# gregorgebhardt/gym-kilobots

Measured on AMD Instinct MI355X. Metric: kilobot-steps/sec, higher is better.
Workload: dtype f32

## Files before the change

### gym_kilobots_amd/csrc/kb_regsolve_bins.inc

```
{
    constexpr int KRB = KB_KREG_BINS;
    const bool solving = (int)__builtin_amdgcn_readfirstlane(wave) < nsolve;
    unsigned ra[KRB], rb[KRB], rm[KRB];
    float racc[KRB], rnx[KRB], rny[KRB];
    const unsigned WOFF = 8u * (unsigned)(NB - 5);
    char *const velB = reinterpret_cast<char *>(vel), *const posB = reinterpret_cast<char *>(pos);
#define RB_WALL(j) (ra[j] >= WOFF)
#define RB_WALLIDX(j) ((int)((ra[j] - WOFF) >> 3))
#define RB_VEL(off) (*reinterpret_cast<float2 *>(velB + (off)))
#define RB_POS(off) (*reinterpret_cast<float2 *>(posB + (off)))
#define RB_C(j) ((int)(rm[j] & 0xFFFu))
#define RB_DEPTH(j) ((int)((rm[j] >> 12) & 0x1FFu))
#define RB_FLIP(j) (((rm[j] >> 21) & 1u) != 0u)
#define RB_ISL(j) ((int)(rm[j] >> 22))
#pragma unroll
    for (int j = 0; j < KRB; ++j) { ra[j] = 0u; rb[j] = 0u; rm[j] = 0u; racc[j] = 0.0f; rnx[j] = 1.0f; rny[j] = 0.0f; }
    unsigned long long slotLevels[KRB];
    int dlo[KRB], dhi[KRB];
#pragma unroll
    for (int j = 0; j < KRB; ++j) { slotLevels[j] = 0ull; dlo[j] = 1; dhi[j] = 0; }
    int maxD = 0;
    unsigned mycnt = 0;
    const float nm_bb = p.nm_bb, nm_wb = p.nm_wb;
    const int DUMMY = NB - 1;
#ifdef KB_SOLVER_PRIO
    __builtin_amdgcn_s_setprio(KB_SOLVER_PRIO);
#endif
    if (solving) {
        unsigned mybase = 0;
        for (int w = 0; w < wave; ++w) mybase += misc[M_WCNT + w];
        mycnt = misc[M_WCNT + wave];
        unsigned lk[KRB];
        unsigned lp[KRB];
        int rdepth[KRB];
#define RB_A(j) ((int)(lp[j] & 0xFFFFu))
#define RB_B(j) ((int)(lp[j] >> 16))
        unsigned mlo = 0, mhi = 0;
#pragma unroll
        for (int j = 0; j < KRB; ++j) {
            const unsigned idx = lane + 64u * j;
            lk[j] = 0u; lp[j] = 0u; rdepth[j] = 0;
            if (idx < mycnt) {
                const unsigned c = lOrder[mybase + idx];
                const unsigned pr = lPair[c], inf = lInfo[c];
                const unsigned cls = inf & 0x7Fu, r = (inf >> 8) & 0xFFu;
                lp[j] = pr;
                unsigned key = cls * RK + (r < RK - 1 ? r : RK - 1);
                if (SLEEP && !active[parent[pr >> 16]]) key = 63u;
                else {
                    if (key < 32u) mlo |= 1u << key; else mhi |= 1u << (key - 32u);
                    if (r >= RK - 1) atomicMax(&bkMaxRank[wave * NUM_CLS + cls], r);
                }
                lk[j] = key | (r << 8) | (c << 16) | 0x80000000u;
            }
        }
        mlo = wave_or(mlo); mhi = wave_or(mhi);
        const unsigned long long keymask = ((unsigned long long)mhi << 32) | mlo;
        wave_sync();
#ifdef KB_PROFILE
        if (tid == 0) { atomicAdd(&KB_PROF(8), (unsigned)__popcll(keymask)); atomicAdd(&KB_PROF(11), 1u); }
#endif
        KB_STAMP_PRE(19);
        unsigned *bodyDepth = islCnt;
        {
            auto depth_round = [&](unsigned key_, int r_) __attribute__((always_inline)) {
                int ia[KRB], ib[KRB];
                unsigned da[KRB], db[KRB];
                bool on[KRB];
#pragma unroll
                for (int j = 0; j < KRB; ++j) {
                    on[j] = (lk[j] >> 31) && (lk[j] & 63u) == key_ && (r_ < 0 || (int)((lk[j] >> 8) & 0xFFu) == r_);
                    ia[j] = (on[j] && RB_A(j) < WALL_CODE) ? RB_A(j) : DUMMY;
                    ib[j] = on[j] ? RB_B(j) : DUMMY;
                    da[j] = bodyDepth[ia[j]]; db[j] = bodyDepth[ib[j]];
                }
#pragma unroll
                for (int j = 0; j < KRB; ++j) {
                    const unsigned d = max((on[j] && RB_A(j) < WALL_CODE) ? da[j] : 0u, db[j]) + 1u;
                    if (on[j]) {
                        rdepth[j] = (int)d;
                        bodyDepth[ib[j]] = d;
                        if (RB_A(j) < WALL_CODE) bodyDepth[ia[j]] = d;
                    }
                }
                wave_sync();
            };
            for (unsigned long long m_ = keymask; m_; m_ &= m_ - 1) {
                const unsigned key_ = (unsigned)__builtin_ctzll(m_);
                if ((key_ % RK) < RK - 1) depth_round(key_, -1);
                else {
                    const int maxr_ = (int)bkMaxRank[wave * NUM_CLS + key_ / RK];
                    for (int r_ = RK - 1; r_ <= maxr_; ++r_) depth_round(key_, r_);
                }
            }
        }
#pragma unroll
        for (int j = 0; j < KRB; ++j) maxD = max(maxD, rdepth[j]);
        maxD = (int)wave_umax((unsigned)maxD);
        KB_STAMP_PRE(20);
        if (mycnt > 64u) {
            unsigned base_ = 0;
            for (int d_ = SLEEP ? 0 : 1; d_ <= maxD; ++d_) {
#pragma unroll
                for (int j = 0; j < KRB; ++j) {
                    const bool is = (lk[j] >> 31) && rdepth[j] == d_;
                    const unsigned long long m_ = __ballot(is);
                    if (is) {
                        const unsigned at = mybase + base_ + (unsigned)__popcll(m_ & ((1ull << lane) - 1ull));
                        lOrder[at] = (unsigned short)((lk[j] >> 16) & 0xFFFu);
                        lCbk[at] = (unsigned short)d_;
                    }
                    base_ += (unsigned)__popcll(m_);
                }
            }
            wave_sync();
#pragma unroll
            for (int j = 0; j < KRB; ++j)
                if (lk[j] >> 31) { lk[j] = (lk[j] & 0x8000FFFFu) | ((unsigned)lOrder[mybase + lane + 64u * j] << 16); rdepth[j] = lCbk[mybase + lane + 64u * j]; }
        }
        KB_STAMP_PRE(21);
#pragma unroll
        for (int j = 0; j < KRB; ++j) {
            const unsigned long long mine = (lk[j] >> 31) ? 1ull << min(rdepth[j], 63) : 0ull;
            const unsigned lo = wave_or((unsigned)mine), hi = wave_or((unsigned)(mine >> 32));
            slotLevels[j] = ((unsigned long long)hi << 32) | (unsigned long long)lo;
            const unsigned long long lv = slotLevels[j] >> 1;
            dlo[j] = lv ? (int)__builtin_ctzll(lv) + 1 : 1;
            dhi[j] = lv ? ((lv >> 62) ? maxD : 64 - (int)__builtin_clzll(lv)) : 0;
        }
#pragma unroll
        for (int j = 0; j < KRB; ++j) {
            ra[j] = 0u; rb[j] = 0u; rm[j] = 0u;
            if (lk[j] >> 31) {
                const unsigned c = (lk[j] >> 16) & 0xFFFu;
                const unsigned pr = lPair[c], inf = lInfo[c];
                const int a = (int)(pr & 0xFFFFu), b = (int)(pr >> 16);
                const bool flip = (inf & 0x80u) != 0u;
                ra[j] = a >= WALL_CODE ? WOFF + 8u * (unsigned)(a - WALL_CODE) : 8u * (unsigned)a;
                rb[j] = 8u * (unsigned)b;
                racc[j] = lAcc[c];
                rm[j] = c | ((unsigned)rdepth[j] << 12) | (flip ? 1u << 21 : 0u) | (parent[b] << 22);
                if (a >= WALL_CODE) {
                    float dist, nx, ny;
                    wall_geom(p, a - WALL_CODE, pos[b].x, pos[b].y, dist, nx, ny);
                    if (flip) { nx = -nx; ny = -ny; }
                    rnx[j] = nx; rny[j] = ny;
                } else {
                    const float dx = pos[b].x - pos[a].x, dy = pos[b].y - pos[a].y;
                    const float dd = dx * dx + dy * dy;
                    if (dd > B2_EPSILON * B2_EPSILON) {
                        const float len = sqrtf(dd);
                        const float inv = 1.0f / len;
                        rnx[j] = dx * inv; rny[j] = dy * inv;
                    }
                }
            }
        }
#undef RB_A
#undef RB_B
#ifdef KB_PROFILE
        if (lane == 0) atomicMax(&misc[M_PROF], (unsigned)maxD);
        if (tid == 0) atomicAdd(&KB_PROF(M_PROF_DEPTH), (unsigned)maxD);
        KB_STAMP(7);
#endif
    }
    KB_ABLATE_EXIT(9);
#define RB_ON(j) (RB_DEPTH(j) == d_)
    if (solving) {
#pragma unroll
        for (int j = 0; j < KRB; ++j) {
            for (int d_ = dlo[j]; d_ <= dhi[j]; ++d_) {
                if (RB_ON(j)) {
                    const float2 va = RB_VEL(ra[j]), vb = RB_VEL(rb[j]);
                    const float Px = racc[j] * rnx[j], Py = racc[j] * rny[j];
                    const float ima = RB_WALL(j) ? 0.0f : p.im_bot;
                    RB_VEL(ra[j]) = make_float2(va.x - ima * Px, va.y - ima * Py);
                    RB_VEL(rb[j]) = make_float2(vb.x + p.im_bot * Px, vb.y + p.im_bot * Py);
                }
                wave_sync();
            }
        }
        KB_STAMP_PRE(29);
    }
    KB_ABLATE_EXIT(10);
    if (solving) {
        for (int it = 0; it < p.vel_iters; ++it) {
#pragma unroll
            for (int j = 0; j < KRB; ++j) {
                for (int d_ = dlo[j]; d_ <= dhi[j]; ++d_) {
                    if (RB_ON(j)) {
                        const float2 va = RB_VEL(ra[j]), vb = RB_VEL(rb[j]);
                        const bool wallA = RB_WALL(j);
                        const float nx = rnx[j], ny = rny[j];
                        const float ima = wallA ? 0.0f : p.im_bot, imb = p.im_bot;
                        const float dvx = vb.x - va.x, dvy = vb.y - va.y;
                        const float vn = dvx * nx + dvy * ny;
                        float lambda = -((wallA ? nm_wb : nm_bb) * vn);
                        const float accOld = racc[j];
                        const float newimp = fmaxf(accOld + lambda, 0.0f);
                        lambda = newimp - accOld;
                        racc[j] = newimp;
                        const float Px = lambda * nx, Py = lambda * ny;
                        RB_VEL(ra[j]) = make_float2(va.x - ima * Px, va.y - ima * Py);
                        RB_VEL(rb[j]) = make_float2(vb.x + imb * Px, vb.y + imb * Py);
                    }
                    wave_sync();
                }
            }
        }
        KB_STAMP_PRE(30);
    }
#ifdef KB_SOLVER_PRIO
    __builtin_amdgcn_s_setprio(0);
#endif
    __syncthreads();
    KB_STAMP(4);
    KB_RETID();
    KB_ABLATE_EXIT(11);
#ifdef KB_PROFILE
    if (tid == 0) atomicAdd(&KB_PROF(9), misc[M_PROF]);
#endif
    if (solving) {
#pragma unroll
        for (int j = 0; j < KRB; ++j)
            if (lane + 64u * j < mycnt) lAcc[RB_C(j)] = racc[j];
    }
#pragma unroll
    for (int q = 0; q < BPT; ++q) {
        const int b_ = tid + q * nt;
        if (b_ >= N) continue;
        const int b = ms[q];
        float vxx = vel[b].x, vyy = vel[b].y, ww = bw[q];
        startX[b] = pos[b].x; startY[b] = pos[b].y;
        const float tx = h * vxx, ty = h * vyy;
        if (tx * tx + ty * ty > B2_MAX_TRANSLATION_SQ) {
            const float ratio = B2_MAX_TRANSLATION / sqrtf(tx * tx + ty * ty);
            vxx *= ratio; vyy *= ratio;
        }
        const float rot = h * ww;
        if (rot * rot > B2_MAX_ROTATION_SQ) {
            const float ratio = B2_MAX_ROTATION / fabsf(rot);
            ww *= ratio;
        }
        pos[b].x += h * vxx; pos[b].y += h * vyy;
        th[q] += h * ww;
        vel[b].x = vxx; vel[b].y = vyy; bw[q] = ww;
        if (SLEEP) islWave[b] = (unsigned char)((active[b] ? 2 : 0) | (p.pos_iters <= 0 ? 1 : 0));
    }
    __syncthreads();
    KB_STAMP(5);
    KB_RETID();
    KB_ABLATE_EXIT(12);
    if (solving) {
#ifdef KB_SOLVER_PRIO
        __builtin_amdgcn_s_setprio(KB_SOLVER_PRIO);
#endif
        for (int it = 0; it < p.pos_iters; ++it) {
            unsigned char *act = active + (it & 1) * NB, *nxt = active + ((it + 1) & 1) * NB;
            bool viol = false;
            bool ron[KRB];
#pragma unroll
            for (int j = 0; j < KRB; ++j) ron[j] = (lane + 64u * j < mycnt) && act[RB_ISL(j)] != 0;
#pragma unroll
            for (int j = 0; j < KRB; ++j) {
                for (int d_ = dlo[j]; d_ <= dhi[j]; ++d_) {
                    if (ron[j] && RB_ON(j)) {
                    const bool wallA = RB_WALL(j);
                    const int isl = RB_ISL(j);
                    float nx, ny, sep;
                    const float ima = wallA ? 0.0f : p.im_bot, imb = p.im_bot;
                    const float2 pb = RB_POS(rb[j]);
                    const float bx = pb.x, by = pb.y;
                    float axx = 0.0f, ayy = 0.0f;
                    if (wallA) {
                        float dist, wx, wy;
                        wall_geom(p, RB_WALLIDX(j), bx, by, dist, wx, wy);
                        nx = RB_FLIP(j) ? -wx : wx; ny = RB_FLIP(j) ? -wy : wy;
                        const float along = RB_FLIP(j) ? -dist : dist;
                        sep = along - B2_POLYGON_RADIUS - p.r_bot;
                    } else {
                        const float2 pa = RB_POS(ra[j]);
                        axx = pa.x; ayy = pa.y;
                        const float dx = bx - axx, dy = by - ayy;
                        const float dd = dx * dx + dy * dy;
                        if (__builtin_expect(__builtin_amdgcn_ballot_w64(!kb_exact_guard(dd)) == 0ull, 1)) {
                            const float len = kb_sqrt_refine(dd, __builtin_amdgcn_sqrtf(dd), __builtin_amdgcn_rsqf(dd));
                            const float inv = kb_rcp_refine(len, __builtin_amdgcn_rcpf(len));
                            nx = dx * inv; ny = dy * inv;
                        } else {
                            const float len = sqrtf(dd);
                            nx = dx; ny = dy;
                            if (!(len < B2_EPSILON)) { const float inv = 1.0f / len; nx = dx * inv; ny = dy * inv; }
                        }
                        sep = (dx * nx + dy * ny) - p.r_bot - p.r_bot;
                    }
                    if (sep < -3.0f * B2_LINEAR_SLOP) { nxt[isl] = 1; viol = true; if (SLEEP && it == p.pos_iters - 1) islWave[isl] = 3; }
                    const float C = kb_clampf(B2_BAUMGARTE * (sep + B2_LINEAR_SLOP), -B2_MAX_LINEAR_CORRECTION, 0.0f);
                    const float K = ima + imb;
                    const float imp = __builtin_expect(p.exact_div, 1) ? kb_div_const(-C, K, wallA ? p.y_wb : p.y_bb) : (K > 0.0f ? -C / K : 0.0f);
                    const float Px = imp * nx, Py = imp * ny;
                    if (!wallA) RB_POS(ra[j]) = make_float2(axx - ima * Px, ayy - ima * Py);
                    RB_POS(rb[j]) = make_float2(bx + imb * Px, by + imb * Py);
                    }
                    wave_sync();
                }
            }
#ifdef KB_PROFILE
            if (tid == 0) atomicAdd(&KB_PROF(10), 1u);
#endif
            if (!__any(viol)) break;
#pragma unroll
            for (int j = 0; j < KRB; ++j) if (lane + 64u * j < mycnt) act[RB_ISL(j)] = 0;
            wave_sync();
        }
        KB_STAMP_PRE(24);
#ifdef KB_SOLVER_PRIO
        __builtin_amdgcn_s_setprio(0);
#endif
    }
#undef RB_WALL
#undef RB_WALLIDX
#undef RB_VEL
#undef RB_POS
#undef RB_C
#undef RB_DEPTH
#undef RB_FLIP
#undef RB_ISL
#undef RB_ON
}
```

### gym_kilobots_amd/csrc/kb_step_kernel.h

```cpp
#pragma once
#include <utility>

#include "kb_common.h"
#include "kb_objects.h"

namespace kb {

template <int DRIVE_MODE, int LIGHT_TYPE, bool OBJ, int FN = 0, int TIER = 0, bool POLY = true, bool SENSE = true, bool SLEEP = false>
__global__ void __launch_bounds__(TIER == 1 ? 64 : 64 * KB_MAX_WAVES, (TIER == 1 || TIER == 3) ? 2 : ((TIER == 2 || (FN != 0 && !OBJ)) ? KB_COMPACT_WAVES_PER_SIMD : KB_MIN_WAVES_PER_SIMD)) kb_step_kernel(const Params p) {
    constexpr bool WIDE = TIER == 1 || TIER == 3;
    constexpr bool BINS = !OBJ;
    constexpr int KRX = BINS ? KB_KREG_BINS : KREG;
    constexpr bool PAR_DS = FN != 0 && BINS;
    static_assert(!SLEEP || FN == 0 || !OBJ, "the fixed-size instantiations with objects do not carry the sleep state");
    extern __shared__ __align__(16) unsigned char smem[];
    int e = blockIdx.x;
    int tid = threadIdx.x;
    const int nt = FN ? 64 * KB_MAX_WAVES : (int)blockDim.x;
    int lane = tid & 63, wave = tid >> 6;
    const int wave_s = __builtin_amdgcn_readfirstlane(wave);
    const int nw = nt >> 6;
    const int nsolve = BINS ? (nw >= KB_NSOLVE_DIV ? nw / KB_NSOLVE_DIV : 1) : nw;
    const int N = FN ? FN : p.N, NP = FN ? ((FN + 3) & ~3) : p.NP, S = p.S;
    size_t o = (size_t)e * N;
// ... 947 lines not shown
                        int rbase = 0;
                        for (unsigned a2 = head[hix(cell)]; a2 != (unsigned)EMPTY16; a2 = nextb[a2])
                            if ((int)a2 < a && (!hashed || (int)cellOf[a2] == cell)) rbase += (int)((dirCnt[a2] >> (6 * k)) & 63u);
                        int j = 0;
                        if (((dc >> (6 * k)) & 63u) > 1u) {
                            const int oc = (cy + dir_dy(k)) * p.gw + (cx + dir_dx(k));
                            for (unsigned b2 = head[hix(oc)]; b2 != (unsigned)EMPTY16; b2 = nextb[b2]) {
                                if (b2 >= b || (k == 0 && (int)b2 <= a) || (hashed && (int)cellOf[b2] != oc)) continue;
                                const float2 pb2 = pos[b2];
                                const float ex = pb2.x - ax, ey = pb2.y - ay;
                                if (!(ex * ex + ey * ey > rr2)) j++;
                            }
                        }
                        r = rbase + j;
                        slot = sbase + j;
                        acc = ws_find(a, b);
                        if (acc < 0.0f) acc = ws_find((int)b, (unsigned)a);
                        unsigned ra = a, rb = b;
                        for (;;) {
                            while (true) { unsigned t = lds_load_relaxed<PAR_DS>(&parent[ra]); if (t == ra) break; ra = t; }
                            while (true) { unsigned t = lds_load_relaxed<PAR_DS>(&parent[rb]); if (t == rb) break; rb = t; }
                            if (ra == rb) break;
                            if (ra < rb) { unsigned t = ra; ra = rb; rb = t; }
                            if (atomicCAS(&parent[ra], ra, rb) == ra) break;
                        }
                    }
                    if (acc < 0.0f) acc = 0.0f;
                    if (slot >= S) slot = 255;
                    if (r > 255) { r = 255; atomicOr(&misc[M_STATUS], 4u); }
                    sInfo[c] = (unsigned)cls | ((unsigned)r << 8) | ((unsigned)slot << 16) | fixbits;
                    sAcc[c] = acc;
                }
            };
            if (big) label_pass(gPair, gInfo, gAcc); else label_pass(lPair, lInfo, lAcc);
            KB_STAMP_PRE(18);
            __syncthreads();
            KB_STAMP(2);
            KB_RETID();

        }

        if (SLEEP) {
#pragma unroll
            for (int q = 0; q < BPT; ++q) {
                const int b = tid + q * nt;
                if (b >= N) continue;
                const int cnt = wsCnt[b], off = wsOff[b];
                for (int s_ = 0; s_ < cnt && off + s_ < p.cap; ++s_) {
                    const float a_ = oldInLds ? oldAcc[off + s_] : g.ws_acc[wo + off + s_];
                    if (a_ < 0.0f) continue;
                    unsigned key = oldInLds ? (unsigned)oldKey[off + s_] : g.ws_key[wo + off + s_];
                    if (!oldInLds) key = key >= KEY_OBJ ? OBJ_CODE + (key - KEY_OBJ) : (key >= KEY_WALL ? WALL_CODE + (key - KEY_WALL) : key);
                    if (key >= (unsigned)WALL_CODE) continue;
                    if (slp[q] < 0.0f) slp[q] = 0.0f;
                    if (key >= (unsigned)OBJ_CODE) {
                        if (OBJ) { const int m_ = ot_body(objTab + (key - OBJ_CODE) * OT_WORDS); if (objSlp[m_] < 0.0f) objSlp[m_] = 0.0f; }
                    } else atomicOr(&misc[M_WAKE + (key >> 5)], 1u << (key & 31u));
                }
            }
            __syncthreads();
#pragma unroll
            for (int q = 0; q < BPT; ++q) {
                const int b = tid + q * nt;
                if (b < N && slp[q] < 0.0f && ((misc[M_WAKE + (b >> 5)] >> (b & 31)) & 1u)) slp[q] = 0.0f;
            }
        }
        for (int b = tid; b < N; b += nt) {
            unsigned r = b;
            while (true) { unsigned t = lds_load_relaxed<PAR_DS>(&parent[r]); if (t == r) break; r = t; }
            parent[b] = r;
            islCnt[b] = 0;
            islWave[b] = (unsigned char)((unsigned)b % (unsigned)nsolve);
            if (!BINS) head[hix(cellOf[b])] = EMPTY16;
            if (!SLEEP) active[b] = 1;
            active[NB + b] = 0;
            if (!BINS && SENSE && p.sense_s > 0 && drive) g.nbr_count[o + b] = (unsigned)newOff[b];
        }
        if (tid < 64) bkStart[tid] = 0;
        if (tid < 32) bkFill[tid] = 0;
        if (tid < M) {
            const int b = N + tid;
            unsigned r = b;
            while (true) { unsigned t = lds_load_relaxed<PAR_DS>(&parent[r]); if (t == r) break; r = t; }
            parent[b] = r;
            islCnt[b] = 0;
            islWave[b] = (unsigned char)((unsigned)b % (unsigned)nw);
            if (!SLEEP) active[b] = 1;
            active[NB + b] = 0;
        }
        if (SLEEP && !BINS) {
#pragma unroll
            for (int q = 0; q < BPT; ++q) {
                const int b = tid + q * nt;
                if (b < N && !(slp[q] < 0.0f)) active[parent[b]] = 1;
            }
            if (tid < M && !(objSlp[tid] < 0.0f)) active[parent[N + tid]] = 1;
        }
        if (BINS) __syncthreads();
        else newTotal = block_scan_u8(wsCntNew, newOff, NP, wsum, tid);
        if (SLEEP && BINS) {
#pragma unroll
            for (int q = 0; q < BPT; ++q) {
                const int b = tid + q * nt;
                if (b < N && !(slp[q] < 0.0f)) active[parent[ms[q]]] = 1;
            }
        }
        const bool newInLds = BINS ? !big : newTotal <= (unsigned)capL_;
        if (OBJ && wave == 0) {
            unsigned root = 0;
            const bool on = lane < NMC && mcTouch;
            if (on) { root = parent[mci(ox, MC_B, lane)]; mci_set(ox, MC_ISL, lane, (int)root); }
        }
        KB_STAMP(14);
        KB_RETID();
        KB_ABLATE_EXIT(7);
        const bool wcntDead = BINS && nw > 1 && p.solver_mode == 0;
        auto census = [&](const unsigned *sPair) __attribute__((always_inline)) {
            for (int c = tid; c < ncon; c += nt) {
                const unsigned root = parent[sPair[c] >> 16];
                const unsigned n = atomicAdd(&islCnt[root], 1u) + 1u;
                if (n > (unsigned)GIANT_ISLAND) atomicMax(&misc[M_MAXISL], n);
                if (!wcntDead) atomicAdd(&misc[M_WCNT + islWave[root]], 1u);
            }
        };
        if (big) census(gPair); else census(lPair);
        __syncthreads();
        unsigned maxw = 0;
        for (int w = 0; w < nw; ++w) maxw = max(maxw, misc[M_WCNT + w]);
        bool coopForced = misc[M_MAXISL] > (unsigned)GIANT_ISLAND || p.solver_mode == 2 || p.solver_mode == 4;
        bool coop = coopForced || nw == 1;
        if (!coop && !big && p.solver_mode == 0) {
            unsigned *szSum = bkStart, *szPre = bkStart + 32, *szFill = bkFill;
            for (int b = tid; b < N + M; b += nt) {
                if (parent[b] != (unsigned)b) continue;
                const unsigned cnt_ = islCnt[b];
                if (cnt_ != 0) atomicAdd(&szSum[32u - min(cnt_, 32u)], cnt_);
            }
            __syncthreads();
            if (wave == 0) {
                const unsigned v_ = lane < 32 ? szSum[lane] : 0u;
                const unsigned incl = wave_incl_scan(v_);
                if (lane < 32) szPre[lane] = incl - v_;
                if (lane < nw) misc[M_WCNT + lane] = 0;
            }
            __syncthreads();
            unsigned chunk = 60u;
            if ((unsigned)ncon > 60u * (unsigned)(nw - 1) + 124u) chunk = ((unsigned)ncon - 124u + (unsigned)nw - 2u) / (unsigned)(nw - 1);
            if (BINS) chunk = ((unsigned)ncon + (unsigned)nsolve - 1u) / (unsigned)nsolve;
            for (int b = tid; b < N + M; b += nt) {
                if (parent[b] != (unsigned)b) continue;
                const unsigned cnt_ = islCnt[b];
                if (cnt_ == 0) continue;
                const unsigned q_ = 32u - min(cnt_, 32u);
                const unsigned at = szPre[q_] + atomicAdd(&szFill[q_], cnt_);
                const unsigned w_ = min(at / max(chunk, 1u), (unsigned)nsolve - 1u);
                islWave[b] = (unsigned char)w_;
                atomicAdd(&misc[M_WCNT + w_], cnt_);
            }
            __syncthreads();
            maxw = 0;
            for (int w = 0; w < nw; ++w) maxw = max(maxw, misc[M_WCNT + w]);
        }
        bool reg = !coopForced && !big && maxw <= 64u * KRX && p.solver_mode == 0;
        if (!coop && !big && maxw > 64u * KRX && p.solver_mode == 0) {
            unsigned short *bigList = bkList;
            __syncthreads();
            if (tid < nw) misc[M_WCNT + tid] = 0;
            if (tid == 0) misc[M_TOTAL] = 0;
            __syncthreads();
            for (int b = tid; b < N + M; b += nt) {
                if (parent[b] != (unsigned)b) continue;
                const unsigned cnt_ = islCnt[b];
                if (cnt_ == 0) continue;
                unsigned slot_ = 64u;
                if (cnt_ >= (unsigned)BIG_ISLAND) slot_ = atomicAdd(&misc[M_TOTAL], 1u);
                if (slot_ < 64u) bigList[slot_] = (unsigned short)b;
                else atomicAdd(&misc[M_WCNT + islWave[b]], cnt_);
            }
            __syncthreads();
            if (wave == 0) {
                const int nb = (int)min(misc[M_TOTAL], 64u);
                const unsigned root = lane < nb ? (unsigned)bigList[lane] : 0u;
                const unsigned size = lane < nb ? islCnt[root] : 0u;
                int rank = 0;
                for (int j = 0; j < nb; ++j) {
                    const unsigned sj = __shfl(size, j), rj = __shfl(root, j);
                    if (sj > size || (sj == size && rj < root)) rank++;
                }
                unsigned load = lane < nsolve ? misc[M_WCNT + lane] : 0u;
                int myWave = 0;
                for (int r = 0; r < nb; ++r) {
                    const int src = __builtin_ctzll(__ballot(lane < nb && rank == r));
                    const unsigned sz = __shfl(size, src);
                    unsigned key = lane < nsolve ? ((load << 4) | (unsigned)lane) : 0xFFFFFFFFu;
                    for (int d = 8; d >= 1; d >>= 1) key = min(key, __shfl_xor(key, d));
                    const int wmin = (int)(__shfl(key, 0) & 15u);
                    if (lane == wmin) load += sz;
                    if (lane == src) myWave = wmin;
                }
                if (lane < nb) islWave[root] = (unsigned char)myWave;
                if (lane < nsolve) misc[M_WCNT + lane] = load;
            }
            __syncthreads();
            maxw = 0;
            for (int w = 0; w < nw; ++w) maxw = max(maxw, misc[M_WCNT + w]);
            reg = maxw <= 64u * KRX;
        }
        if (BINS && nw > 1 && !reg && p.solver_mode == 0) { coopForced = true; coop = true; }
        if (OBJ && wave == 0) {
            const bool on = lane < NMC && mcTouch && (!SLEEP || active[mci(ox, MC_ISL, lane)] != 0);
            const unsigned w_ = on ? (unsigned)islWave[mci(ox, MC_ISL, lane)] : 0u;
            for (int w = 0; w < nw; ++w) {
                const unsigned long long mk = __ballot(on && (int)w_ == w);
                if (lane == 0) mcMask[w] = mk;
            }
            const unsigned long long all = __ballot(on);
            if (lane == 0) mcMask[nw] = all;
        }
        auto mc_warm_pass = [&](unsigned long long mask, bool leader) __attribute__((always_inline)) {
            if (leader) for (unsigned long long m_ = mask; m_; m_ &= m_ - 1) mc_warm_start(ox, __builtin_ctzll(m_));
        };
        auto mc_velocity_pass = [&](unsigned long long mask, bool leader) __attribute__((always_inline)) {
            if (leader) for (unsigned long long m_ = mask; m_; m_ &= m_ - 1) mc_solve_velocity(ox, __builtin_ctzll(m_));
        };
        auto mc_position_pass = [&](unsigned long long mask, bool leader, const unsigned char *act, unsigned char *nxt, bool lastIt) __attribute__((always_inline)) -> bool {
            bool viol = false;
            if (leader)
                for (unsigned long long m_ = mask; m_; m_ &= m_ - 1) {
                    const int t = __builtin_ctzll(m_);
                    const int isl = mci(ox, MC_ISL, t);
                    if (!act[isl]) continue;
                    const float minSep = mc_solve_position(ox, t, B2_BAUMGARTE);
                    if (minSep < -3.0f * B2_LINEAR_SLOP) { nxt[isl] = 1; viol = true; if (SLEEP && lastIt) islWave[isl] = 3; }
                }
            return viol;
        };
        auto mc_clear_flags = [&](unsigned long long mask, bool leader, unsigned char *act) __attribute__((always_inline)) {
            if (leader) for (unsigned long long m_ = mask; m_; m_ &= m_ - 1) act[mci(ox, MC_ISL, __builtin_ctzll(m_))] = 0;
        };
        auto mc_store = [&]() __attribute__((always_inline)) {
            if (OBJ && wave == 0 && lane < NMC) {
                int owner, col;
                mc_candidate(F, lane, owner, col);
                float *dst = owsMine + (owner * KB_OWS_COLS + col) * KB_OWS_WORDS;
                float o[KB_OWS_WORDS] = {-1.0f, -1.0f, -1.0f, -1.0f, -1.0f, -1.0f};
                if (mcTouch) {
                    const int cnt = (mci(ox, MC_TYPE, lane) >> 2) & 3, ids = mci(ox, MC_ID, lane);
                    o[0] = (float)(ids & 255); o[1] = mcf(ox, MC_NI0, lane); o[2] = mcf(ox, MC_TI0, lane);
                    if (cnt == 2) { o[3] = (float)((ids >> 8) & 255); o[4] = mcf(ox, MC_NI1, lane); o[5] = mcf(ox, MC_TI1, lane); }
                }
#pragma unroll
                for (int k = 0; k < KB_OWS_WORDS; ++k) dst[k] = o[k];
            }
        };
        auto bucket_sort = [&](const unsigned *sPair, const unsigned *sInfo, unsigned short *cbk,
                               unsigned short *order) __attribute__((always_inline)) {
            const int W = coop ? 1 : nw;
            for (int b = tid; b < N + M; b += nt) islCnt[b] = 0;
            for (int k = tid; k < W * BK_PER_WAVE; k += nt) { bkStart[k] = 0; bkFill[k] = 0; }
            for (int k = tid; k < W * NUM_CLS; k += nt) bkMaxRank[k] = 0;
            if (tid == 0) bkStart[W * BK_PER_WAVE] = 0;
            __syncthreads();
            for (int c = tid; c < ncon; c += nt) {
                const unsigned root = parent[sPair[c] >> 16];
                if (SLEEP && !active[root]) { cbk[c] = EMPTY16; continue; }
                const int w = coop ? 0 : (int)islWave[root];
                const unsigned inf = sInfo[c];
                const int cls = inf & 0x7F, r = (inf >> 8) & 0xFF;
                const int bk = (w * NUM_CLS + cls) * RK + (r < RK - 1 ? r : RK - 1);
                cbk[c] = (unsigned short)bk;
                atomicAdd(&bkStart[bk], 1u);
                if (r >= RK - 1) atomicMax(&bkMaxRank[w * NUM_CLS + cls], (unsigned)r);
            }
            __syncthreads();
            if (wave == 0) {
                const int nb = W * BK_PER_WAVE;
                const int chunk = (nb + 63) / 64;
                const int s0 = lane * chunk, e0 = min(nb, s0 + chunk);
                unsigned sum = 0;
                for (int i = s0; i < e0; ++i) sum += bkStart[i];
                const unsigned incl = wave_incl_scan(sum);
                unsigned run = incl - sum;
                for (int i = s0; i < e0; ++i) { unsigned v = bkStart[i]; bkStart[i] = run; run += v; }
                if (lane == 63) bkStart[nb] = incl;
            }
            __syncthreads();
            for (int c = tid; c < ncon; c += nt) {
                const int bk = cbk[c];
                if (SLEEP && bk == (int)EMPTY16) continue;
                order[bkStart[bk] + atomicAdd(&bkFill[bk], 1u)] = (unsigned short)c;
            }
            if (wave < W) {
                const int base = wave * BK_PER_WAVE;
                const bool ne = lane < BK_PER_WAVE && bkStart[base + lane + 1] > bkStart[base + lane];
                const unsigned long long m = __ballot(ne);
                if (ne) bkList[base + __popcll(m & ((1ull << lane) - 1ull))] = (unsigned short)(base + lane);
                if (lane == 0) nList[wave] = (unsigned char)__popcll(m);
            }
            __syncthreads();
        };
        if (reg) {
            for (int b = tid; b < N + M; b += nt) islCnt[b] = 0;
            if (tid < nw * NUM_CLS) bkMaxRank[tid] = 0;
            for (int c = tid; c < ncon; c += nt) {
                const unsigned w = islWave[parent[lPair[c] >> 16]];
                unsigned base = 0;
                for (unsigned w2 = 0; w2 < w; ++w2) base += misc[M_WCNT + w2];
                lOrder[base + atomicAdd(&misc[M_WFILL + w], 1u)] = (unsigned short)c;
            }
            __syncthreads();
        } else if (big) bucket_sort(gPair, gInfo, gCbk, gOrder);
        else bucket_sort(lPair, lInfo, lCbk, lOrder);
        KB_STAMP(3);
        KB_RETID();
        KB_ABLATE_EXIT(8);

        const bool coopLevels = BINS && coopForced && nw > 1;
        if constexpr (BINS) {
            if (reg) {
#include "kb_regsolve_bins.inc"
            } else if (coopLevels) {
#include "kb_coopsolve_bins.inc"
            }
        }
        if (BINS && (reg || coopLevels)) {
        } else if (reg) {
            unsigned mybase = 0;
            for (int w = 0; w < wave; ++w) mybase += misc[M_WCNT + w];
            const unsigned mycnt = misc[M_WCNT + wave];
            int ra[KREG], rb[KREG], rkey[KREG], rrank[KREG], rslot[KREG], risl[KREG], rc[KREG], rdepth[KREG];
            float racc[KREG], rnx[KREG], rny[KREG], rima[KREG], rimb[KREG], rra[KREG], rrb[KREG], rnm[KREG];
            bool rvalid[KREG], rflip[KREG];
            bool rpoly[KREG];
            float rrAx[KREG], rrAy[KREG], rlnx[KREG], rlny[KREG], rlpx[KREG], rlpy[KREG];
            unsigned mlo = 0, mhi = 0;
            const float nm_bb = p.nm_bb, nm_wb = p.nm_wb;
#define R_IMA(j) (OBJ ? rima[j] : (ra[j] < WALL_CODE ? p.im_bot : 0.0f))
#define R_IMB(j) (OBJ ? rimb[j] : p.im_bot)
#define R_RA(j) (OBJ ? rra[j] : (ra[j] < WALL_CODE ? p.r_bot : B2_POLYGON_RADIUS))
#define R_RB(j) (OBJ ? rrb[j] : p.r_bot)
#define R_NM(j) (OBJ ? rnm[j] : (ra[j] < WALL_CODE ? nm_bb : nm_wb))
#pragma unroll
            for (int j = 0; j < KREG; ++j) {
                const unsigned idx = lane + 64u * j;
                rvalid[j] = idx < mycnt;
                ra[j] = 0; rb[j] = 0; rkey[j] = 0; rrank[j] = 0; rc[j] = 0; rdepth[j] = 0;
                if (rvalid[j]) {
                    const int c = lOrder[mybase + idx];
                    const unsigned pr = lPair[c], inf = lInfo[c];
                    const int cls = inf & 0x7F, r = (inf >> 8) & 0xFF;
                    rc[j] = c; ra[j] = pr & 0xFFFF; rb[j] = pr >> 16; rrank[j] = r;
                    const int key = cls * RK + (r < RK - 1 ? r : RK - 1);
                    if (SLEEP && !active[parent[rb[j]]]) {
                        rkey[j] = -1;
                    } else {
                        rkey[j] = key;
                        if (key < 32) mlo |= 1u << key; else mhi |= 1u << (key - 32);
                        if (r >= RK - 1) atomicMax(&bkMaxRank[wave * NUM_CLS + cls], (unsigned)r);
                    }
                }
            }
            mlo = wave_or(mlo); mhi = wave_or(mhi);
            const unsigned long long keymask = ((unsigned long long)mhi << 32) | mlo;
            wave_sync();
#ifdef KB_PROFILE
            if (tid == 0) { atomicAdd(&KB_PROF(8), (unsigned)__popcll(keymask)); atomicAdd(&KB_PROF(11), 1u); }
#endif

#define KB_REG_KEY_ROUNDS(...)                                                                      \
            for (unsigned long long m_ = keymask; m_; m_ &= m_ - 1) {                               \
                const int key_ = __builtin_ctzll(m_);                                               \
                if ((key_ % RK) < RK - 1) {                                                         \
                    _Pragma("unroll") for (int j = 0; j < KREG; ++j)                                \
                        if (rvalid[j] && rkey[j] == key_) { __VA_ARGS__ }                           \
                    wave_sync();                                                                    \
                } else {                                                                            \
                    const int maxr_ = (int)bkMaxRank[wave * NUM_CLS + key_ / RK];                   \
                    for (int r_ = RK - 1; r_ <= maxr_; ++r_) {                                      \
                        _Pragma("unroll") for (int j = 0; j < KREG; ++j)                            \
                            if (rvalid[j] && rkey[j] == key_ && rrank[j] == r_) { __VA_ARGS__ }     \
                        wave_sync();                                                                \
                    }                                                                               \
                }                                                                                   \
            }

            KB_STAMP_PRE(19);
            unsigned *bodyDepth = islCnt;
            {
                const int DUMMYD = NB - 1;
                auto depth_round = [&](int key_, int r_) __attribute__((always_inline)) {
                    int ia[KREG], ib[KREG];
                    unsigned da[KREG], db[KREG];
                    bool on[KREG];
#pragma unroll
                    for (int j = 0; j < KREG; ++j) {
                        on[j] = rvalid[j] && rkey[j] == key_ && (r_ < 0 || rrank[j] == r_);
                        ia[j] = (on[j] && ra[j] < WALL_CODE) ? ra[j] : DUMMYD;
                        ib[j] = on[j] ? rb[j] : DUMMYD;
                        da[j] = bodyDepth[ia[j]]; db[j] = bodyDepth[ib[j]];
                    }
#pragma unroll
                    for (int j = 0; j < KREG; ++j) {
                        const unsigned d = max((on[j] && ra[j] < WALL_CODE) ? da[j] : 0u, db[j]) + 1u;
                        if (on[j]) {
                            rdepth[j] = (int)d;
                            bodyDepth[ib[j]] = d;
                            if (ra[j] < WALL_CODE) bodyDepth[ia[j]] = d;
                        }
                    }
                    wave_sync();
                };
                for (unsigned long long m_ = keymask; m_; m_ &= m_ - 1) {
                    const int key_ = __builtin_ctzll(m_);
                    if ((key_ % RK) < RK - 1) depth_round(key_, -1);
                    else {
                        const int maxr_ = (int)bkMaxRank[wave * NUM_CLS + key_ / RK];
                        for (int r_ = RK - 1; r_ <= maxr_; ++r_) depth_round(key_, r_);
                    }
                }
            }
            int maxD = 0;
#pragma unroll
            for (int j = 0; j < KREG; ++j) maxD = max(maxD, rdepth[j]);
            maxD = (int)wave_umax((unsigned)maxD);
            KB_STAMP_PRE(20);
            if (KREG > 1 && mycnt > 64u) {
                unsigned base_ = 0;
                for (int d_ = SLEEP ? 0 : 1; d_ <= maxD; ++d_) {
#pragma unroll
                    for (int j = 0; j < KREG; ++j) {
                        const bool is = rvalid[j] && rdepth[j] == d_;
                        const unsigned long long m_ = __ballot(is);
                        if (is) {
                            const unsigned at = mybase + base_ + (unsigned)__popcll(m_ & ((1ull << lane) - 1ull));
                            lOrder[at] = (unsigned short)rc[j];
                            lCbk[at] = (unsigned short)d_;
                        }
                        base_ += (unsigned)__popcll(m_);
                    }
                }
                wave_sync();
#pragma unroll
                for (int j = 0; j < KREG; ++j)
                    if (rvalid[j]) { rc[j] = lOrder[mybase + lane + 64u * j]; rdepth[j] = lCbk[mybase + lane + 64u * j]; }
            }
            KB_STAMP_PRE(21);
            unsigned long long slotLevels[KREG];
#pragma unroll
            for (int j = 0; j < KREG; ++j) {
                const unsigned long long mine = rvalid[j] ? 1ull << min(rdepth[j], 63) : 0ull;
                const unsigned lo = wave_or((unsigned)mine), hi = wave_or((unsigned)(mine >> 32));
                slotLevels[j] = ((unsigned long long)hi << 32) | (unsigned long long)lo;
            }
            int dlo[KREG], dhi[KREG];
#pragma unroll
            for (int j = 0; j < KREG; ++j) {
                const unsigned long long lv = slotLevels[j] >> 1;
                dlo[j] = lv ? (int)__builtin_ctzll(lv) + 1 : 1;
                dhi[j] = lv ? ((lv >> 62) ? maxD : 64 - (int)__builtin_clzll(lv)) : 0;
            }
            const bool anyContact = (unsigned)__builtin_amdgcn_readfirstlane((int)mycnt) > 0u;
            constexpr bool FULLMASK = OBJ && !WIDE;
            const int cSafe = (FULLMASK && anyContact) ? (int)lOrder[mybase] : 0;
#pragma unroll
            for (int j = 0; j < KREG; ++j) {
                ra[j] = 0; rb[j] = 0; rslot[j] = 255; risl[j] = 0;
                racc[j] = 0.0f; rnx[j] = 1.0f; rny[j] = 0.0f; rflip[j] = false;
                rima[j] = 0.0f; rimb[j] = 0.0f; rra[j] = 0.0f; rrb[j] = 0.0f; rnm[j] = 0.0f;
                rpoly[j] = false; rrAx[j] = 0.0f; rrAy[j] = 0.0f; rlnx[j] = 0.0f; rlny[j] = 0.0f; rlpx[j] = 0.0f; rlpy[j] = 0.0f;
                if (FULLMASK ? anyContact : rvalid[j]) {
                    const int c = (FULLMASK && !rvalid[j]) ? cSafe : rc[j];
                    const unsigned pr = lPair[c], inf = lInfo[c];
                    const int a = pr & 0xFFFF, b = pr >> 16;
                    ra[j] = a; rb[j] = b; rslot[j] = (inf >> 16) & 0xFF; racc[j] = lAcc[c];
                    rflip[j] = (inf & 0x80) != 0;
                    risl[j] = (int)parent[b];
                    if (OBJ) {
                        rima[j] = bim(a); rimb[j] = bim(b); rra[j] = brad(a); rrb[j] = brad(b);
                        const float k_ = rima[j] + rimb[j];
                        rnm[j] = k_ > 0.0f ? 1.0f / k_ : 0.0f;
                    }
                    if (bpoly(b)) {
                        const float *T = objTab + ((inf >> 24) & 15u) * OT_WORDS;
                        const XF xo = body_xf(ox, b);
                        const V2 bc = mk2(pos[a].x, pos[a].y);
                        V2 ln = mk2(0.0f, 0.0f), lp = mk2(0.0f, 0.0f);
                        collide_poly_circle(T, xo, bc, p.r_bot, ln, lp);
                        const V2 normal = rot_mul(xo, ln);
                        const V2 planePoint = xf_mul(xo, lp);
                        const V2 cA = v_add(bc, v_scale(T[OT_RADIUS] - v_dot(v_sub(bc, planePoint), normal), normal));
                        const V2 cB = v_sub(bc, v_scale(p.r_bot, normal));
                        const V2 point = v_scale(0.5f, v_add(cA, cB));
                        const V2 rA = v_sub(point, mk2(pos[b].x, pos[b].y));
                        const float rnA = v_cross(rA, normal);
                        const float kNormal = T[OT_IM] + KB_IM_BOT(a) + T[OT_II] * rnA * rnA;
                        rpoly[j] = true; rnx[j] = normal.x; rny[j] = normal.y; rrAx[j] = rA.x; rrAy[j] = rA.y;
                        rlnx[j] = ln.x; rlny[j] = ln.y; rlpx[j] = lp.x; rlpy[j] = lp.y;
                        rnm[j] = kNormal > 0.0f ? 1.0f / kNormal : 0.0f;
                    } else if (a >= WALL_CODE) {
                        float dist, nx, ny;
                        wall_geom(p, a - WALL_CODE, pos[b].x, pos[b].y, dist, nx, ny);
                        if (rflip[j]) { nx = -nx; ny = -ny; }
                        rnx[j] = nx; rny[j] = ny;
                    } else {
                        const float dx = pos[b].x - pos[a].x, dy = pos[b].y - pos[a].y;
                        const float dd = dx * dx + dy * dy;
                        if (dd > B2_EPSILON * B2_EPSILON) {
                            const float len = sqrtf(dd);
                            const float inv = 1.0f / len;
                            rnx[j] = dx * inv; rny[j] = dy * inv;
                        }
                    }
                    if (FULLMASK && !rvalid[j]) {
                        ra[j] = 0; rb[j] = 0; rslot[j] = 255; risl[j] = 0;
                        racc[j] = 0.0f; rnx[j] = 1.0f; rny[j] = 0.0f; rflip[j] = false;
                        rima[j] = 0.0f; rimb[j] = 0.0f; rra[j] = 0.0f; rrb[j] = 0.0f; rnm[j] = 0.0f;
                        rpoly[j] = false; rrAx[j] = 0.0f; rrAy[j] = 0.0f; rlnx[j] = 0.0f; rlny[j] = 0.0f; rlpx[j] = 0.0f; rlpy[j] = 0.0f;
                    }
                }
            }
#ifdef KB_PROFILE
            if (lane == 0) atomicMax(&misc[M_PROF], (unsigned)maxD);
            if (tid == 0) atomicAdd(&KB_PROF(M_PROF_DEPTH), (unsigned)maxD);
            KB_STAMP(7);
#endif
#define KB_REG_ROUNDS(...)                                                                          \
            _Pragma("unroll") for (int j = 0; j < KREG; ++j)                                        \
                for (int d_ = dlo[j]; d_ <= dhi[j]; ++d_) {                                         \
                    if (rvalid[j] && rdepth[j] == d_) { __VA_ARGS__ }                               \
                    wave_sync();                                                                    \
                }

            KB_ABLATE_EXIT(9);
            unsigned long long myMc = 0ull;
            if (OBJ) {
                const unsigned long long mm = mcMask[wave];
                myMc = ((unsigned long long)(unsigned)__builtin_amdgcn_readfirstlane((unsigned)(mm >> 32)) << 32) |
                       (unsigned long long)(unsigned)__builtin_amdgcn_readfirstlane((unsigned)mm);
                myMc &= NMC >= 64 ? ~0ull : ((1ull << NMC) - 1ull);
            }
            KB_REG_ROUNDS({
                const int a = ra[j], b = rb[j];
                const float Px = racc[j] * rnx[j], Py = racc[j] * rny[j];
                if (OBJ && rpoly[j]) {
                    const int m = b - N;
                    objW[m] -= objBody[m * BT_WORDS + BT_II] * (rrAx[j] * Py - rrAy[j] * Px);
                    vel[b].x -= R_IMB(j) * Px; vel[b].y -= R_IMB(j) * Py;
                    vel[a].x += R_IMA(j) * Px; vel[a].y += R_IMA(j) * Py;
                } else {
                    if (a < WALL_CODE) { vel[a].x -= R_IMA(j) * Px; vel[a].y -= R_IMA(j) * Py; }
                    vel[b].x += R_IMB(j) * Px; vel[b].y += R_IMB(j) * Py;
                }
            })
            if (OBJ && myMc) { mc_warm_pass(myMc, lane == 0); wave_sync(); }
            KB_STAMP_PRE(29);
            KB_ABLATE_EXIT(10);
            const int DUMMY = NB - 1;
            for (int it = 0; it < p.vel_iters; ++it) {
#pragma unroll
                for (int j = 0; j < KREG; ++j) {
                    for (int d_ = dlo[j]; d_ <= dhi[j]; ++d_) {
                        if (rvalid[j] && rdepth[j] == d_) {
                            if (OBJ && rpoly[j]) {
                                const int a = ra[j], b = rb[j], m = b - N;
                                const float wA = objW[m];
                                const float dvx = (vel[a].x - vel[b].x) - (-wA * rrAy[j]), dvy = (vel[a].y - vel[b].y) - (wA * rrAx[j]);
                                const float vn = dvx * rnx[j] + dvy * rny[j];
                                float lambda = -(rnm[j] * vn);
                                const float accOld = racc[j];
                                const float newimp = fmaxf(accOld + lambda, 0.0f);
                                lambda = newimp - accOld;
                                racc[j] = newimp;
                                const float Px = lambda * rnx[j], Py = lambda * rny[j];
                                vel[b].x -= rimb[j] * Px; vel[b].y -= rimb[j] * Py;
                                objW[m] = wA - objBody[m * BT_WORDS + BT_II] * (rrAx[j] * Py - rrAy[j] * Px);
                                vel[a].x += rima[j] * Px; vel[a].y += rima[j] * Py;
                            } else {
                                const bool wallA = ra[j] >= WALL_CODE;
                                const int ia = wallA ? DUMMY : ra[j], ib = rb[j];
                                const float2 va_ = vel[ia], vb_ = vel[ib];
                                const float nx = rnx[j], ny = rny[j];
                                const float ima = R_IMA(j), imb = R_IMB(j);
                                const float ax_ = wallA ? 0.0f : va_.x, ay_ = wallA ? 0.0f : va_.y;
                                const float dvx = vb_.x - ax_, dvy = vb_.y - ay_;
                                const float vn = dvx * nx + dvy * ny;
                                float lambda = -(R_NM(j) * vn);
                                const float accOld = racc[j];
                                const float newimp = fmaxf(accOld + lambda, 0.0f);
                                lambda = newimp - accOld;
                                racc[j] = newimp;
                                const float Px = lambda * nx, Py = lambda * ny;
                                vel[ia] = make_float2(ax_ - ima * Px, ay_ - ima * Py);
                                vel[ib] = make_float2(vb_.x + imb * Px, vb_.y + imb * Py);
                            }
                        }
                        wave_sync();
                    }
                }
                if (OBJ && myMc) { mc_velocity_pass(myMc, lane == 0); wave_sync(); }
            }
            KB_STAMP_PRE(30);
            __syncthreads();
            KB_STAMP(4);
            KB_RETID();
            KB_ABLATE_EXIT(11);
            mc_store();
#ifdef KB_PROFILE
            if (tid == 0) atomicAdd(&KB_PROF(9), misc[M_PROF]);
#endif
            const bool last = sub == p.n_substeps - 1;
#pragma unroll
// ... 723 lines not shown
```

Before: 16.13 billion.

## Restructure register solver setup: batched loads, prefix-scan wave bases, lighter depth rounds

Replaces per-thread serial prefix sums of per-wave counts with a single wave scan that seeds M_WFILL, so bucketing and wave base lookup need no loops. The register-solver setup batches its LDS loads across slots, precomputes a packed key/rank code and byte offsets for the depth rounds, and skips slots past the first when no later slot holds that key. Bank max-rank is read by readlane, and reorder writes are deferred using mbcnt. Pair normals use fast sqrt/rcp with refinement behind a wave-wide exactness guard. This adds code complexity and relies on the M_WFILL semantics changing consistently.

```diff
diff --git a/gym_kilobots_amd/csrc/kb_regsolve_bins.inc b/gym_kilobots_amd/csrc/kb_regsolve_bins.inc
--- a/gym_kilobots_amd/csrc/kb_regsolve_bins.inc
+++ b/gym_kilobots_amd/csrc/kb_regsolve_bins.inc
@@ -22,40 +22,63 @@
     int maxD = 0;
     unsigned mycnt = 0;
     const float nm_bb = p.nm_bb, nm_wb = p.nm_wb;
-    const int DUMMY = NB - 1;
 #ifdef KB_SOLVER_PRIO
     __builtin_amdgcn_s_setprio(KB_SOLVER_PRIO);
 #endif
     if (solving) {
-        unsigned mybase = 0;
-        for (int w = 0; w < wave; ++w) mybase += misc[M_WCNT + w];
         mycnt = misc[M_WCNT + wave];
+        const unsigned mybase = misc[M_WFILL + wave] - mycnt;
         unsigned lk[KRB];
         unsigned lp[KRB];
         int rdepth[KRB];
+        unsigned klo[KRB], khi[KRB];
 #define RB_A(j) ((int)(lp[j] & 0xFFFFu))
 #define RB_B(j) ((int)(lp[j] >> 16))
-        unsigned mlo = 0, mhi = 0;
-#pragma unroll
-        for (int j = 0; j < KRB; ++j) {
-            const unsigned idx = lane + 64u * j;
-            lk[j] = 0u; lp[j] = 0u; rdepth[j] = 0;
-            if (idx < mycnt) {
-                const unsigned c = lOrder[mybase + idx];
-                const unsigned pr = lPair[c], inf = lInfo[c];
-                const unsigned cls = inf & 0x7Fu, r = (inf >> 8) & 0xFFu;
-                lp[j] = pr;
+        {
+            unsigned c_[KRB], inf_[KRB];
+            bool v_[KRB], awake_[KRB];
+#pragma unroll
+            for (int j = 0; j < KRB; ++j) {
+                const unsigned idx = lane + 64u * j;
+                v_[j] = idx < mycnt;
+                c_[j] = lOrder[v_[j] ? mybase + idx : 0u];
+            }
+#pragma unroll
+            for (int j = 0; j < KRB; ++j) {
+                c_[j] = v_[j] ? c_[j] : 0u;
+                lp[j] = lPair[c_[j]]; inf_[j] = lInfo[c_[j]];
+            }
+#pragma unroll
+            for (int j = 0; j < KRB; ++j) { lp[j] = v_[j] ? lp[j] : 0u; awake_[j] = true; }
+            if (SLEEP) {
+                unsigned root_[KRB];
+#pragma unroll
+                for (int j = 0; j < KRB; ++j) root_[j] = parent[lp[j] >> 16];
+#pragma unroll
+                for (int j = 0; j < KRB; ++j) awake_[j] = active[root_[j]] != 0;
+            }
+#pragma unroll
+            for (int j = 0; j < KRB; ++j) {
+                const unsigned cls = inf_[j] & 0x7Fu, r = (inf_[j] >> 8) & 0xFFu;
                 unsigned key = cls * RK + (r < RK - 1 ? r : RK - 1);
-                if (SLEEP && !active[parent[pr >> 16]]) key = 63u;
-                else {
-                    if (key < 32u) mlo |= 1u << key; else mhi |= 1u << (key - 32u);
-                    if (r >= RK - 1) atomicMax(&bkMaxRank[wave * NUM_CLS + cls], r);
-                }
-                lk[j] = key | (r << 8) | (c << 16) | 0x80000000u;
-            }
-        }
-        mlo = wave_or(mlo); mhi = wave_or(mhi);
-        const unsigned long long keymask = ((unsigned long long)mhi << 32) | mlo;
+                const bool on = v_[j] && awake_[j];
+                if (!on) key = 63u;
+                const unsigned bit = on ? 1u << (key & 31u) : 0u;
+                klo[j] = key < 32u ? bit : 0u; khi[j] = key < 32u ? 0u : bit;
+                if (on && r >= RK - 1) atomicMax(&bkMaxRank[wave * NUM_CLS + cls], r);
+                lk[j] = v_[j] ? (key | (r << 8) | (c_[j] << 16) | 0x80000000u) : 0u;
+                rdepth[j] = 0;
+            }
+        }
+        unsigned long long keymask = 0ull, restmask = 0ull;
+        {
+            unsigned mlo = 0, mhi = 0, rlo = 0, rhi = 0;
+#pragma unroll
+            for (int j = 0; j < KRB; ++j) { mlo |= klo[j]; mhi |= khi[j]; if (j > 0) { rlo |= klo[j]; rhi |= khi[j]; } }
+            mlo = wave_or(mlo); mhi = wave_or(mhi);
+            keymask = ((unsigned long long)mhi << 32) | mlo;
+            if (mycnt > 64u) { rlo = wave_or(rlo); rhi = wave_or(rhi); restmask = ((unsigned long long)rhi << 32) | rlo; }
+        }
         wave_sync();
 #ifdef KB_PROFILE
         if (tid == 0) { atomicAdd(&KB_PROF(8), (unsigned)__popcll(keymask)); atomicAdd(&KB_PROF(11), 1u); }
@@ -63,60 +86,81 @@
         KB_STAMP_PRE(19);
         unsigned *bodyDepth = islCnt;
         {
-            auto depth_round = [&](unsigned key_, int r_) __attribute__((always_inline)) {
-                int ia[KRB], ib[KRB];
-                unsigned da[KRB], db[KRB];
-                bool on[KRB];
-#pragma unroll
-                for (int j = 0; j < KRB; ++j) {
-                    on[j] = (lk[j] >> 31) && (lk[j] & 63u) == key_ && (r_ < 0 || (int)((lk[j] >> 8) & 0xFFu) == r_);
-                    ia[j] = (on[j] && RB_A(j) < WALL_CODE) ? RB_A(j) : DUMMY;
-                    ib[j] = on[j] ? RB_B(j) : DUMMY;
-                    da[j] = bodyDepth[ia[j]]; db[j] = bodyDepth[ib[j]];
-                }
-#pragma unroll
-                for (int j = 0; j < KRB; ++j) {
-                    const unsigned d = max((on[j] && RB_A(j) < WALL_CODE) ? da[j] : 0u, db[j]) + 1u;
-                    if (on[j]) {
-                        rdepth[j] = (int)d;
-                        bodyDepth[ib[j]] = d;
-                        if (RB_A(j) < WALL_CODE) bodyDepth[ia[j]] = d;
-                    }
-                }
-                wave_sync();
-            };
+            char *const bdB = reinterpret_cast<char *>(bodyDepth);
+#define RB_BD(off) (*reinterpret_cast<unsigned *>(bdB + (off)))
+            unsigned rc[KRB], ia4[KRB], ib4[KRB];
+#pragma unroll
+            for (int j = 0; j < KRB; ++j) {
+                const unsigned key = lk[j] & 63u, r = (lk[j] >> 8) & 0xFFu;
+                const bool on = (lk[j] >> 31) != 0u && key != 63u;
+                rc[j] = on ? ((key % RK) == RK - 1 ? (key | (r << 6)) : key) : 0xFFFFFFFFu;
+                ib4[j] = 4u * (unsigned)RB_B(j);
+                ia4[j] = RB_A(j) < WALL_CODE ? 4u * (unsigned)RB_A(j) : ib4[j];
+            }
+            const unsigned mrow = bkMaxRank[wave * NUM_CLS + min((int)lane, NUM_CLS - 1)];
             for (unsigned long long m_ = keymask; m_; m_ &= m_ - 1) {
                 const unsigned key_ = (unsigned)__builtin_ctzll(m_);
-                if ((key_ % RK) < RK - 1) depth_round(key_, -1);
+                const bool rest_ = ((restmask >> key_) & 1ull) != 0ull;
+                auto depth_round = [&](unsigned code_) __attribute__((always_inline)) {
+#pragma unroll
+                    for (int j = 0; j < KRB; ++j) {
+                        if (j == 0 || rest_) {
+                            if (rc[j] == code_) {
+                                const unsigned d = max(RB_BD(ia4[j]), RB_BD(ib4[j])) + 1u;
+                                rdepth[j] = (int)d;
+                                RB_BD(ib4[j]) = d;
+                                RB_BD(ia4[j]) = d;
+                            }
+                        }
+                    }
+                    wave_sync();
+                };
+                if ((key_ % RK) < RK - 1) depth_round(key_);
                 else {
-                    const int maxr_ = (int)bkMaxRank[wave * NUM_CLS + key_ / RK];
-                    for (int r_ = RK - 1; r_ <= maxr_; ++r_) depth_round(key_, r_);
-                }
-            }
+                    const unsigned maxr_ = (unsigned)__builtin_amdgcn_readlane((int)mrow, (int)(key_ / RK));
+                    for (unsigned r_ = RK - 1; r_ <= maxr_; ++r_) depth_round(key_ | (r_ << 6));
+                }
+            }
+#undef RB_BD
         }
 #pragma unroll
         for (int j = 0; j < KRB; ++j) maxD = max(maxD, rdepth[j]);
         maxD = (int)wave_umax((unsigned)maxD);
         KB_STAMP_PRE(20);
         if (mycnt > 64u) {
+            unsigned at[KRB];
+#pragma unroll
+            for (int j = 0; j < KRB; ++j) at[j] = 0u;
             unsigned base_ = 0;
             for (int d_ = SLEEP ? 0 : 1; d_ <= maxD; ++d_) {
 #pragma unroll
                 for (int j = 0; j < KRB; ++j) {
                     const bool is = (lk[j] >> 31) && rdepth[j] == d_;
                     const unsigned long long m_ = __ballot(is);
-                    if (is) {
-                        const unsigned at = mybase + base_ + (unsigned)__popcll(m_ & ((1ull << lane) - 1ull));
-                        lOrder[at] = (unsigned short)((lk[j] >> 16) & 0xFFFu);
-                        lCbk[at] = (unsigned short)d_;
-                    }
+                    const unsigned mine = __builtin_amdgcn_mbcnt_hi((unsigned)(m_ >> 32), __builtin_amdgcn_mbcnt_lo((unsigned)m_, base_));
+                    at[j] = is ? mine : at[j];
                     base_ += (unsigned)__popcll(m_);
                 }
             }
+#pragma unroll
+            for (int j = 0; j < KRB; ++j)
+                if (lk[j] >> 31) {
+                    lOrder[mybase + at[j]] = (unsigned short)((lk[j] >> 16) & 0xFFFu);
+                    lCbk[mybase + at[j]] = (unsigned short)rdepth[j];
+                }
             wave_sync();
-#pragma unroll
-            for (int j = 0; j < KRB; ++j)
-                if (lk[j] >> 31) { lk[j] = (lk[j] & 0x8000FFFFu) | ((unsigned)lOrder[mybase + lane + 64u * j] << 16); rdepth[j] = lCbk[mybase + lane + 64u * j]; }
+            unsigned short o_[KRB], l_[KRB];
+#pragma unroll
+            for (int j = 0; j < KRB; ++j) {
+                const unsigned i_ = mybase + ((lk[j] >> 31) ? lane + 64u * j : 0u);
+                o_[j] = lOrder[i_]; l_[j] = lCbk[i_];
+            }
+#pragma unroll
+            for (int j = 0; j < KRB; ++j) {
+                const bool v_ = (lk[j] >> 31) != 0u;
+                lk[j] = v_ ? ((lk[j] & 0x8000FFFFu) | ((unsigned)o_[j] << 16)) : lk[j];
+                rdepth[j] = v_ ? (int)l_[j] : rdepth[j];
+            }
         }
         KB_STAMP_PRE(21);
 #pragma unroll
@@ -128,31 +172,56 @@
             dlo[j] = lv ? (int)__builtin_ctzll(lv) + 1 : 1;
             dhi[j] = lv ? ((lv >> 62) ? maxD : 64 - (int)__builtin_clzll(lv)) : 0;
         }
-#pragma unroll
-        for (int j = 0; j < KRB; ++j) {
-            ra[j] = 0u; rb[j] = 0u; rm[j] = 0u;
-            if (lk[j] >> 31) {
-                const unsigned c = (lk[j] >> 16) & 0xFFFu;
-                const unsigned pr = lPair[c], inf = lInfo[c];
-                const int a = (int)(pr & 0xFFFFu), b = (int)(pr >> 16);
-                const bool flip = (inf & 0x80u) != 0u;
-                ra[j] = a >= WALL_CODE ? WOFF + 8u * (unsigned)(a - WALL_CODE) : 8u * (unsigned)a;
+        {
+            unsigned c_[KRB], pr_[KRB], inf_[KRB], root_[KRB];
+            float acc_[KRB];
+            float2 pa_[KRB], pb_[KRB];
+            bool v_[KRB];
+#pragma unroll
+            for (int j = 0; j < KRB; ++j) {
+                v_[j] = (lk[j] >> 31) != 0u;
+                c_[j] = v_[j] ? (lk[j] >> 16) & 0xFFFu : 0u;
+                pr_[j] = lPair[c_[j]]; inf_[j] = lInfo[c_[j]]; acc_[j] = lAcc[c_[j]];
+            }
+#pragma unroll
+            for (int j = 0; j < KRB; ++j) {
+                pr_[j] = v_[j] ? pr_[j] : 0u;
+                const int a = (int)(pr_[j] & 0xFFFFu), b = (int)(pr_[j] >> 16);
+                pa_[j] = pos[a >= WALL_CODE ? b : a]; pb_[j] = pos[b]; root_[j] = parent[b];
+            }
+            bool pairOn[KRB];
+            float dx[KRB], dy[KRB], dd[KRB], wnx[KRB], wny[KRB];
+            bool ieee = false;
+#pragma unroll
+            for (int j = 0; j < KRB; ++j) {
+                const int a = (int)(pr_[j] & 0xFFFFu), b = (int)(pr_[j] >> 16);
+                const bool wallA = a >= WALL_CODE, flip = (inf_[j] & 0x80u) != 0u;
+                ra[j] = wallA ? WOFF + 8u * (unsigned)(a - WALL_CODE) : 8u * (unsigned)a;
                 rb[j] = 8u * (unsigned)b;
-                racc[j] = lAcc[c];
-                rm[j] = c | ((unsigned)rdepth[j] << 12) | (flip ? 1u << 21 : 0u) | (parent[b] << 22);
-                if (a >= WALL_CODE) {
-                    float dist, nx, ny;
-                    wall_geom(p, a - WALL_CODE, pos[b].x, pos[b].y, dist, nx, ny);
-                    if (flip) { nx = -nx; ny = -ny; }
-                    rnx[j] = nx; rny[j] = ny;
-                } else {
-                    const float dx = pos[b].x - pos[a].x, dy = pos[b].y - pos[a].y;
-                    const float dd = dx * dx + dy * dy;
-                    if (dd > B2_EPSILON * B2_EPSILON) {
-                        const float len = sqrtf(dd);
-                        const float inv = 1.0f / len;
-                        rnx[j] = dx * inv; rny[j] = dy * inv;
-                    }
+                racc[j] = v_[j] ? acc_[j] : 0.0f;
+                rm[j] = v_[j] ? (c_[j] | ((unsigned)rdepth[j] << 12) | (flip ? 1u << 21 : 0u) | (root_[j] << 22)) : 0u;
+                float dist;
+                wall_geom(p, wallA ? a - WALL_CODE : 0, pb_[j].x, pb_[j].y, dist, wnx[j], wny[j]);
+                if (flip) { wnx[j] = -wnx[j]; wny[j] = -wny[j]; }
+                dx[j] = pb_[j].x - pa_[j].x; dy[j] = pb_[j].y - pa_[j].y;
+                dd[j] = dx[j] * dx[j] + dy[j] * dy[j];
+                pairOn[j] = v_[j] && !wallA && dd[j] > B2_EPSILON * B2_EPSILON;
+                ieee = ieee || (pairOn[j] && !kb_exact_guard(dd[j]));
+                if (wallA) { rnx[j] = wnx[j]; rny[j] = wny[j]; } else { rnx[j] = 1.0f; rny[j] = 0.0f; }
+            }
+            if (__builtin_expect(__builtin_amdgcn_ballot_w64(ieee) == 0ull, 1)) {
+#pragma unroll
+                for (int j = 0; j < KRB; ++j) {
+                    const float len = kb_sqrt_refine(dd[j], __builtin_amdgcn_sqrtf(dd[j]), __builtin_amdgcn_rsqf(dd[j]));
+                    const float inv = kb_rcp_refine(len, __builtin_amdgcn_rcpf(len));
+                    if (pairOn[j]) { rnx[j] = dx[j] * inv; rny[j] = dy[j] * inv; }
+                }
+            } else {
+#pragma unroll
+                for (int j = 0; j < KRB; ++j) {
+                    const float len = sqrtf(dd[j]);
+                    const float inv = 1.0f / len;
+                    if (pairOn[j]) { rnx[j] = dx[j] * inv; rny[j] = dy[j] * inv; }
                 }
             }
         }
diff --git a/gym_kilobots_amd/csrc/kb_step_kernel.h b/gym_kilobots_amd/csrc/kb_step_kernel.h
--- a/gym_kilobots_amd/csrc/kb_step_kernel.h
+++ b/gym_kilobots_amd/csrc/kb_step_kernel.h
@@ -1273,11 +1273,24 @@
         if (reg) {
             for (int b = tid; b < N + M; b += nt) islCnt[b] = 0;
             if (tid < nw * NUM_CLS) bkMaxRank[tid] = 0;
-            for (int c = tid; c < ncon; c += nt) {
-                const unsigned w = islWave[parent[lPair[c] >> 16]];
-                unsigned base = 0;
-                for (unsigned w2 = 0; w2 < w; ++w2) base += misc[M_WCNT + w2];
-                lOrder[base + atomicAdd(&misc[M_WFILL + w], 1u)] = (unsigned short)c;
+            if constexpr (BINS) {
+                if (wave_s == 0) {
+                    const unsigned v_ = lane < nw ? misc[M_WCNT + lane] : 0u;
+                    const unsigned incl = wave_incl_scan(v_);
+                    if (lane < nw) misc[M_WFILL + lane] = incl - v_;
+                }
+                __syncthreads();
+                for (int c = tid; c < ncon; c += nt) {
+                    const unsigned w = islWave[parent[lPair[c] >> 16]];
+                    lOrder[atomicAdd(&misc[M_WFILL + w], 1u)] = (unsigned short)c;
+                }
+            } else {
+                for (int c = tid; c < ncon; c += nt) {
+                    const unsigned w = islWave[parent[lPair[c] >> 16]];
+                    unsigned base = 0;
+                    for (unsigned w2 = 0; w2 < w; ++w2) base += misc[M_WCNT + w2];
+                    lOrder[base + atomicAdd(&misc[M_WFILL + w], 1u)] = (unsigned short)c;
+                }
             }
             __syncthreads();
         } else if (big) bucket_sort(gPair, gInfo, gCbk, gOrder);
```

Result: faster. 16.39 billion, median of 6 (+1.6%).
